# UoB-HPC/pbf-sph

Hardware: AMD Instinct MI355X
Metric: particle-steps/sec (1 M particles, 4 iters) + achieved HBM GB/s, 1/2/4/8 MI355X (higher is better)
Workload: dtype f32; 1 GPU; dam-break, 1024000 particles (nominal 1048576), box 4600^3, h=0.1, K=4, dt=0.01245, scale=500; timed = simulation frames [200, 2687) after 195 settle + 5 warm-up frames; particles=1024000, solver_iter=4, settle_frames=195, math=precise (IEEE div/sqrt, no contraction), parallelism=1 GPU, device-resident

## Files before the change

### pbf-sph_amd/csrc/pbf_hip.hip

```cpp
#include "pbf_hip.h"

#include <hip/hip_runtime.h>

#include <cmath>
#include <cstdio>
#include <cstdlib>
#include <cstring>
#include <algorithm>
#include <atomic>
#include <initializer_list>
#include <limits>
#include <map>
#include <string>
#include <utility>
#include <vector>

#include "pbf_kernels.hpp"
#include "pbf_slab.hpp"
#include "pbf_tiles.hpp"
#include "pbf_mc.hpp"
#include "pbf_whitewater.hpp"
#include "pbf_anisotropy.hpp"
#include "pbf_aniso_field.hpp"
#include "pbf_mesh_sdf.hpp"
// ... 44 lines not shown
  ~Pinned() { reset(); }
  void reset() {
    if (p) (void)hipHostFree(p);
    p = nullptr, count = 0;
  }
  hipError_t ensure(size_t n, bool zero = true) {
    if (count >= n) return hipSuccess;
    reset();
    const hipError_t e = hipHostMalloc(reinterpret_cast<void **>(&p), n * sizeof(T), hipHostMallocDefault);
    if (e != hipSuccess) {
      p = nullptr;
      return e;
    }
    if (zero) std::memset(static_cast<void *>(p), 0, n * sizeof(T));
    count = n;
    return hipSuccess;
  }
};

template <typename T> struct Mailbox {
  Pinned<T> rec;
  uint32_t seq = 0;
  hipError_t arm(uint32_t &word) {
    word = ++seq ? seq : ++seq;
    return rec.ensure(1);
  }
};
struct SceneRecord {
  uint32_t kept, seq;
};

constexpr uint32_t kTickets = 252;
constexpr uint32_t kCtlWords = kTickets + 4;
constexpr int kBrickZ = 4;

enum Stage { ST_PREDICT = 0, ST_SORT, ST_DIFFUSE, ST_LAMBDA, ST_DELTA, ST_FINALISE, ST_BUILD, ST_COUNT };
const char *kStageNames[ST_COUNT] = {"advect+zindex",      "sortz+gridtable", "sph-diffuse",
                                     "sph-lambda",         "sph-delta",       "sph-finalise",
                                     "sph-lambda/list-build"};

struct EventPair {
  hipEvent_t a, b;
  int stage;
};

}

struct StepState {
  DerivedState st;
  bool hasObstacles;
  uint32_t tableN, gatherSeq;
  uint64_t extent[3];
  double minExtent[3];
  void *bufs[15];
  size_t caps[15];
};
struct GraphEntry {
  hipGraphExec_t exec = nullptr;
  StepState after;
};
struct GraphKey {
  StepState before;
  unsigned char params[sizeof(double) * 11 + 32];
  uint64_t n;
  uint64_t collider;
  int options[10];
// ... 22 lines not shown
  bool ghostsPending = false;
  bool slabConfigured = false;
  pbf_slab_cut slabCut{0, 0, 0, 0};
  uint32_t xoff = 0;
  int32_t shiftL = 0, shiftR = 0;
  pbf_comm *comm = nullptr;
  std::vector<uint32_t> cuts;
  uint32_t capMig = 0, capGhost = 0;
  uint32_t wireCap = 0;
  DevBuf wireSend[2], wireRecv[2];
  DevBuf wireGhost[2];
  bool slabStepMode = false;
  size_t sortLive = 0;
  uint32_t ghostAt = 0;
  uint32_t slabSeq = 0;
  uint64_t slabHostSyncs = 0;
  Pinned<uint32_t> hostCounts;
  size_t reserve = 0;
  uint32_t nOwned = 0, sentL = 0, sentR = 0, gotL = 0, gotR = 0;
  DevBuf latticePN, latticeC, mcCounts, mcOffsets, mcSums, meshV, meshN, meshC, mcNear;
  Pinned<char> meshHost;
  bool meshStaged = false;
  uint64_t mcSample[3] = {0, 0, 0};
  uint64_t mcTriangles = 0;
  DevBuf mcEdgeWord, mcEdgeOffsets, mcEdgeSums, meshT;
  enum MeshKind { MESH_NONE, MESH_SOUP, MESH_INDEXED };
  MeshKind meshKind = MESH_NONE;
  uint64_t mcVertices = 0;
  DevBuf qpos;
  DevBuf nbrList, nbrCount;
  int rowMajor = 1;
  DevBuf rowPstar[2], rowMass, rowQpos, rowXYZ, rowType, rowSlotOf, linTable, linSums;
  DevBuf rowCol, rowMortonOf, rowSegs;
  uint32_t rowSegShift = 0;
  uint32_t diffuseCap = 0;
  int rowDiffuse = 1;
  uint32_t rowShift = 0;
  uint64_t nbrExtraAt = 0;
  uint32_t nbrChunks = 0, nbrChunksOpt = 0;
  double cohesion = 0, adhesion = 0;
  DevBuf surfA, surfB;
  ColliderState col;
  SolidLattice<DevBuf> solid[2];
  DevBuf colliderPose;
  DevBuf pushRec, pushCtl, pushPartials, pushOut;
  Mailbox<WrenchRecord> hostWrench;
  DevBuf bodyRec;
  Mailbox<BodyStateRecord> hostBody;
  DevBuf frictionRec, frictionCtl, frictionPartials;
  Mailbox<WrenchRecord> hostFriction;
  bool sdfCull = true;
  uint64_t sdfLaunchPairs = 0;
  std::vector<pbf_source> sources;
  std::vector<pbf_drain> drains;
  uint32_t emitTotal = 0;
  size_t uploaded = 0;
  DevBuf sceneSources, sceneDrains, drainCounts;
  Mailbox<SceneRecord> hostScene;
  uint64_t sceneHostSyncs = 0;
  DevBuf queryPoints, queryCounts, queryIds;
  DevBuf samplePoints, sampleOut;
  DevBuf diagRho, diagNbr, diagPartials;
  Mailbox<DiagRecord> hostDiag;
  uint64_t diagRhoAt = 0;
  uint64_t orderEpoch = 1;
  bool wwOn = false;
// ... 1 lines not shown
  uint64_t wwFrame = 0;
  size_t wwCount = 0;
  int wwCur = 0;
  DevBuf wwPos[2], wwVel[2], wwKind[2], wwParent[2];
  DevBuf wwSample, wwAlive, wwAliveOff, wwSums, wwFieldA, wwFieldB, wwPot, wwEmit, wwOffset, wwChildKind;
  Mailbox<WwRecord> hostWw;
  uint64_t wwPotAt = 0;
  DevBuf anisoOut;
  DevBuf anisoRec;
  void *regPtr = nullptr;
  size_t regBytes = 0;
  size_t stagedBytes = 0;
  int graphMode = 0;
  std::map<GraphKey, GraphEntry> graphs;
  uint64_t allocEpoch = 0;
  uint32_t graphMisses = 0;
  uint64_t graphReplays = 0, graphCaptures = 0;
  pbf_params lastParams{};
  bool haveParams = false;
  bool reuseLists = true;
  int splitBuild = 8;
  int pipeline = -1;
  int coop = 0;
  bool fusePredict = true;
  bool cellDiffuse = true;
  bool overlapDiffuse = true;
  bool overlapDiffuseForced = false;
  hipStream_t sideStream = nullptr;
  hipStream_t copyStream = nullptr;
  hipEvent_t evPacked = nullptr;
  bool downloadPending = false;
  hipEvent_t evFork = nullptr, evJoin = nullptr;
  bool diffusePending = false;
  DevBuf diffSum, diffCnt;
  bool fuseDiffuse = false;
  bool fuseNextPredict = false;
  DevBuf bricks, brickCtl;
  DevBuf bigCells;
  uint32_t gatherSeq = 0;
  int numCUs = 256;
  uint32_t timingMask = 0xFFFFFFFFu;
  uint32_t padLds = 0;
  std::map<const void *, size_t> ldsLimit;
  int gatherKind = 1;
  uint32_t tileCap = 0, listMax = 0;
  size_t tableCap = 0;
  uint32_t tableN = 0;
  uint64_t extent[3] = {0, 0, 0};
  double minExtent[3] = {0, 0, 0};

  std::vector<EventPair> pending;
  std::vector<hipEvent_t> freeEvents;
  double stageMs[ST_COUNT] = {0};
  uint64_t stageCalls[ST_COUNT] = {0};
};

namespace {

#define HIPCHK(ctx, expr)                                                                          \
  do {                                                                                             \
    hipError_t e_ = (expr);                                                                        \
    if (e_ != hipSuccess) {                                                                        \
      (ctx)->err = std::string(#expr) + ": " + hipGetErrorString(e_);                              \
      return PBF_ERR_HIP;                                                                          \
    }                                                                                              \
  } while (0)

int fail(pbf_ctx *ctx, int code, const std::string &msg) {
  ctx->err = msg;
  return code;
}

int ensure(pbf_ctx *ctx, DevBuf &b, size_t bytes, bool zero = false) {
  if (b.cap >= bytes) return PBF_OK;
  DevBuf fresh;
  fresh.cap = bytes + bytes / 4 + 256;
  HIPCHK(ctx, hipMalloc(&fresh.p, fresh.cap));
  ctx->allocEpoch++;
  if (zero) HIPCHK(ctx, hipMemsetAsync(fresh.p, 0, fresh.cap, ctx->stream));
  if (b.p) {
    HIPCHK(ctx, hipStreamSynchronize(ctx->stream));
    HIPCHK(ctx, b.reset());
  }
  b = std::move(fresh);
  return PBF_OK;
}

bool record_current(const pbf_ctx *ctx, uint64_t madeAt) { return madeAt == ctx->orderEpoch && ctx->st.sorted; }

template <typename N> size_t vsz() { return sizeof(vec4<N>); }

int ensure_particles(pbf_ctx *ctx, size_t n) {
  n = std::max(n, ctx->reserve);
  if (ctx->cap >= n) return PBF_OK;
  if (ctx->reserve) n += n / 4 + 65536;
  const size_t v = ctx->fp64 ? sizeof(double4) : sizeof(float4);
  for (int s = 0; s < 2; ++s) {
    if (int rc = ensure(ctx, ctx->pos4[s], n * v)) return rc;
    if (int rc = ensure(ctx, ctx->vel4[s], n * v)) return rc;
    if (int rc = ensure(ctx, ctx->col4[s], n * v)) return rc;
    if (int rc = ensure(ctx, ctx->id[s], n * 8)) return rc;
    if (int rc = ensure(ctx, ctx->type[s], n)) return rc;
    if (int rc = ensure(ctx, ctx->key[s], n * 4)) return rc;
  }
  for (int s = 0; s < 3; ++s)
    if (int rc = ensure(ctx, ctx->pstar[s], n * v)) return rc;
  if (int rc = ensure(ctx, ctx->permTmp, n * 4)) return rc;
// ... 57 lines not shown
  }
  if (ctx->slabConfigured) {
    c.xoff = ctx->xoff;
    const uint64_t hi = ctx->slabCut.has_right ? std::min<uint64_t>(ext[0], uint64_t(ctx->slabCut.xhi) + 1) : ext[0];
    ext[0] = hi > ctx->xoff ? hi - ctx->xoff : 1;
  }
  c.tableN = morton_encode(uint32_t(ext[0]), uint32_t(ext[1]), uint32_t(ext[2]));
  if (c.tableN == 0) return fail(ctx, PBF_ERR_INVALID, "empty grid (max_bound <= min_bound?)");
  c.poly6Factor = poly6_factor<N>(h);
  c.spikyFactor = spiky_factor<N>(h);
  {
    const N r = N(CorrDeltaQ * h);
    const N d = (h * h) - r * r;
    c.p6DeltaQ = r <= h ? c.poly6Factor * (d * d * d) : N(0);
  }
  c.diffuseT = c.dt / N(750.0);
  c.h2filter = (h * h) * N(1.00001);
  c.n = uint32_t(ctx->n);
  c.nWells = uint32_t(p->n_wells > 0 ? p->n_wells : 0);
  c.hasObstacles = ctx->hasObstacles ? 1u : 0u;
  ctx->tableN = c.tableN;
  return PBF_OK;
}

int drop_histogram(pbf_ctx *ctx) {
  if (ctx->st.counted && ctx->count.p) HIPCHK(ctx, hipMemsetAsync(ctx->count.p, 0, ctx->count.cap, ctx->stream));
  ctx->st.histogram_dropped();
  return PBF_OK;
}

int ensure_table(pbf_ctx *ctx, uint32_t tableN) {
  const size_t entries = size_t(tableN) + 2;
  if (ctx->tableCap >= entries) return PBF_OK;
  if (ctx->count.p) {
    HIPCHK(ctx, hipStreamSynchronize(ctx->stream));
    HIPCHK(ctx, ctx->count.reset());
  }
  if (int rc = ensure(ctx, ctx->count, (entries + SCAN_TILE) * 4, true)) return rc;
  if (int rc = ensure(ctx, ctx->table, (entries + SCAN_TILE) * 4)) return rc;
  const size_t nb = (entries + SCAN_TILE - 1) / SCAN_TILE + 1;
  if (int rc = ensure(ctx, ctx->blockSums, nb * 4)) return rc;
  if (int rc = ensure(ctx, ctx->bricks, (entries / Brick<kBrickZ>::HOME + 2) * 4)) return rc;
  if (int rc = ensure(ctx, ctx->brickCtl, kCtlWords * 4)) return rc;
  ctx->tableCap = ctx->count.cap / 4 - SCAN_TILE;
  return PBF_OK;
}

hipEvent_t get_event(pbf_ctx *ctx) {
  if (!ctx->freeEvents.empty()) {
    hipEvent_t e = ctx->freeEvents.back();
    ctx->freeEvents.pop_back();
    return e;
  }
  hipEvent_t e = nullptr;
  (void)hipEventCreate(&e);
  return e;
}
int resolve_events(pbf_ctx *ctx) {
  if (ctx->pending.empty()) return PBF_OK;
  HIPCHK(ctx, hipStreamSynchronize(ctx->stream));
  for (auto &ep : ctx->pending) {
    float ms = 0.f;
    if (hipEventElapsedTime(&ms, ep.a, ep.b) == hipSuccess) {
      ctx->stageMs[ep.stage] += ms;
      ctx->stageCalls[ep.stage] += 1;
    }
    ctx->freeEvents.push_back(ep.a);
    ctx->freeEvents.push_back(ep.b);
  }
  ctx->pending.clear();
  return PBF_OK;
}
struct StageTimer {
  pbf_ctx *ctx;
  EventPair ep{};
  bool on;
// ... 83 lines not shown
  return PBF_OK;
}

bool row_mode(const pbf_ctx *ctx);

void brick_list(pbf_ctx *ctx, uint32_t tableN, bool counterIsZero = false) {
  if (ctx->st.bricksValid) return;
  if (!counterIsZero) (void)hipMemsetAsync(ctx->brickCtl.p, 0, 4, ctx->stream);
  const uint32_t home = Brick<kBrickZ>::HOME, nBricks = (tableN + home - 1) / home;
  hipLaunchKernelGGL(k_brick_list, grid_for(nBricks), dim3(BLOCK), 0, ctx->stream, ctx->table.as<const uint32_t>(), tableN, home,
                     nBricks, ctx->bricks.as<uint32_t>(), ctx->brickCtl.as<uint32_t>());
  ctx->st.bricks_listed();
}

void launch_scans(pbf_ctx *ctx, const ScanJobs &jobs, int njobs, uint32_t *zero = nullptr, uint32_t nZero = 0) {
  const uint32_t blocks = jobs.nb[0] + (njobs > 1 ? jobs.nb[1] : 0u);
  hipLaunchKernelGGL(k_scan_block_sums, dim3(blocks), dim3(BLOCK), 0, ctx->stream, jobs);
  hipLaunchKernelGGL(k_scan_sums, dim3(uint32_t(njobs)), dim3(BLOCK), 0, ctx->stream, jobs, zero, nZero);
  hipLaunchKernelGGL(k_scan_apply, dim3(blocks), dim3(BLOCK), 0, ctx->stream, jobs);
}
ScanJobs scan_job(const uint32_t *count, uint32_t len, uint32_t *sums, uint32_t *table) {
  ScanJobs j{};
  j.count[0] = count, j.sums[0] = sums, j.table[0] = table, j.len[0] = len, j.nb[0] = (len + SCAN_TILE - 1) / SCAN_TILE;
  return j;
}

int ensure_reaction(pbf_ctx *ctx);
template <typename N> int stage_sort(pbf_ctx *ctx, const pbf_params *p) {
  if (!ctx->st.counted) return fail(ctx, PBF_ERR_STATE, "pbf_stage_sort needs pbf_stage_predict first");
  StepConsts<N> c;
  if (int rc = make_consts<N>(ctx, p, c)) return rc;
  if (c.tableN != ctx->st.countedTableN) return fail(ctx, PBF_ERR_STATE, "bounds changed between predict and sort");
  StageTimer t(ctx, ST_SORT);
  const uint32_t len = c.tableN + 2;
  uint32_t *count = ctx->count.as<uint32_t>(), *table = ctx->table.as<uint32_t>(),
           *sums = ctx->blockSums.as<uint32_t>();
  ScanJobs jobs = scan_job(count, len, sums, table);
  int njobs = 1;
  const int s = ctx->st.cur, d = 1 - s;
  uint32_t *ctl = ctx->brickCtl.as<uint32_t>();
  RowArrays<N> row{};
  const bool rows = row_mode(ctx), rowDiffuse = rows && ctx->cellDiffuse && ctx->rowDiffuse > 0;
  if (rows) {
    uint32_t pshift = 1;
    while (pshift < 10 && (uint64_t(1) << (3 * pshift)) < uint64_t(c.tableN)) ++pshift;
    const size_t ncells = size_t(1) << (3 * pshift), llen = ncells + 1;
    const uint32_t lnb = uint32_t((llen + SCAN_TILE - 1) / SCAN_TILE);
    const size_t v = sizeof(vec4<N>);
    if (int rc = ensure(ctx, ctx->linTable, (ncells + 2 + SCAN_TILE) * 4)) return rc;
    if (int rc = ensure(ctx, ctx->linSums, (size_t(lnb) + 2) * 4)) return rc;
    for (int k = 0; k < 2; ++k)
      if (int rc = ensure(ctx, ctx->rowPstar[k], ctx->cap * v)) return rc;
    if (int rc = ensure(ctx, ctx->rowMass, ctx->cap * sizeof(N))) return rc;
    if (int rc = ensure(ctx, ctx->rowQpos, (ctx->cap + QPOS_PAD) * 8)) return rc;
    if (int rc = ensure(ctx, ctx->rowXYZ, ctx->cap * 4)) return rc;
    if (int rc = ensure(ctx, ctx->rowType, ctx->cap)) return rc;
    if (int rc = ensure(ctx, ctx->rowSlotOf, ctx->cap * 4)) return rc;
    const uint32_t segShift = std::min<uint32_t>(pshift, 6u);
    const size_t nSegTotal = ncells >> segShift;
    if (rowDiffuse) {
      if (int rc = ensure(ctx, ctx->rowCol, ctx->cap * v)) return rc;
      if (int rc = ensure(ctx, ctx->rowMortonOf, ctx->cap * 4)) return rc;
      if (int rc = ensure(ctx, ctx->rowSegs, (std::min(nSegTotal, ctx->cap) + 1) * 4)) return rc;
    }
    jobs.count[1] = nullptr, jobs.rowShift = pshift, jobs.tableN = c.tableN;
    jobs.sums[1] = ctx->linSums.as<uint32_t>(), jobs.table[1] = ctx->linTable.as<uint32_t>();
    jobs.len[1] = uint32_t(llen), jobs.nb[1] = lnb;
    njobs = 2;
    if (rowDiffuse)
      jobs.segs = ctx->rowSegs.as<uint32_t>(), jobs.nSegs = ctl + kTickets + 3, jobs.segShift = segShift;
    launch_scans(ctx, jobs, njobs, ctl, kCtlWords);
    row = RowArrays<N>{ctx->rowPstar[0].as<vec4<N>>(), ctx->rowMass.as<N>(), ctx->rowQpos.as<uint2>(), ctx->rowXYZ.as<uint32_t>(),
                       ctx->rowType.as<uint8_t>(), ctx->rowSlotOf.as<uint32_t>(),
                       rowDiffuse ? ctx->rowCol.as<vec4<N>>() : nullptr, rowDiffuse ? ctx->rowMortonOf.as<uint32_t>() : nullptr,
                       ctx->linTable.as<const uint32_t>(), ctl + kTickets + 2, pshift};
    ctx->rowShift = pshift, ctx->rowSegShift = segShift;
  }
  if (njobs == 1) launch_scans(ctx, jobs, 1, ctl, kCtlWords);
  uint32_t *nBig = ctl + kTickets + 1;
  if (int rc = ensure(ctx, ctx->bigCells, (ctx->cap / BIG_CELL + 2) * 4)) return rc;
  hipLaunchKernelGGL(k_scatter_slots, grid_for(ctx->n), dim3(BLOCK), 0, ctx->stream, c.n, c.tableN,
                     ctx->key[s].as<const uint32_t>(), table, ctx->cellSlot.as<const uint32_t>(), count,
                     ctx->permTmp.as<uint32_t>(),
                     ctx->bigCells.as<uint32_t>(), nBig);
  hipLaunchKernelGGL(k_sort_big_cells, dim3(64), dim3(BLOCK), 0, ctx->stream, table, c.tableN,
                     ctx->bigCells.as<const uint32_t>(), nBig, ctx->permTmp.as<uint32_t>(),
                     ctx->key[s].as<const uint32_t>());
  const size_t nLive = ctx->slabStepMode ? ctx->sortLive : ctx->n;
  hipLaunchKernelGGL((k_rank_move<N>), grid_for(nLive), dim3(BLOCK), 0, ctx->stream, c, uint32_t(nLive), c.tableN,
                     ctx->permTmp.as<const uint32_t>(), table, arrays<N>(ctx, s, s), arrays<N>(ctx, d, d),
                     ctx->slabActive ? ctx->slotOf.as<uint32_t>() : nullptr, ctx->qpos.as<uint2>(), row);
  LAUNCH_CHECK(ctx);
  ctx->n = nLive;
  ctx->gatherSeq = 0;
  ctx->st.sorted_now(rows, rowDiffuse);
  ctx->orderEpoch++;
  if (ctx->col.reaction) {
    if (int rc = ensure_reaction(ctx)) return rc;
    const uint32_t n2 = 2u * uint32_t(ctx->n);
    hipLaunchKernelGGL((k_push_clear<N>), grid_for(std::max<size_t>(n2, 1)), dim3(BLOCK), 0, ctx->stream, n2, ctx->pushRec.as<vec4<N>>(),
                       ctx->pushCtl.as<unsigned long long>());
    LAUNCH_CHECK(ctx);
    ctx->col.records_cleared(ctx->orderEpoch);
  }
  if (!rowDiffuse) brick_list(ctx, c.tableN, true);
  return PBF_OK;
}

inline int other_pstar(const pbf_ctx *ctx) { return ctx->st.pcur == 2 ? ctx->st.cur : 2; }

enum GatherMode { GATHER_PLAIN = 0, GATHER_SAVE_LISTS = 1, GATHER_FROM_LISTS = 2 };

bool row_offsets_fit(const pbf_ctx *ctx) { return uint64_t(ctx->n) * (ctx->fp64 ? sizeof(vec4<double>) : sizeof(vec4<float>)) <= ROW_BYTES_MAX; }
bool row_mode(const pbf_ctx *ctx) {
  return ctx->rowMajor > 0 && ctx->gatherKind == 1 && ctx->splitBuild == 8 && ctx->coop == 0 && ctx->reuseLists &&
         !ctx->fuseDiffuse && ctx->graphMode <= 0 &&
         !(ctx->desc.flags & PBF_FLAG_NO_LDS) && row_offsets_fit(ctx);
}
template <typename N> RowWalk row_walk(pbf_ctx *ctx) {
  return RowWalk{ctx->linTable.as<const uint32_t>(), ctx->rowXYZ.as<const uint32_t>(), ctx->rowSlotOf.as<const uint32_t>(),
                 ctx->table.as<const uint32_t>(), ctx->tableN, ctx->rowShift};
// ... 140 lines not shown
        if (ctx->splitBuild == 4)
          launch_build_lists<N, Lists, 2, 16, FW>(ctx, c, only, ps, qp, args.type, key, table);
        else
          switch (ctx->listMax ? ctx->listMax : 32u) {
            case 16: launch_build_lists<N, Lists, 4, 16, FW>(ctx, c, only, ps, qp, args.type, key, table); break;
            case 24: launch_build_lists<N, Lists, 4, 24, FW>(ctx, c, only, ps, qp, args.type, key, table); break;
            default: launch_build_lists<N, Lists, 4, 32, FW>(ctx, c, only, ps, qp, args.type, key, table); break;
          }
      }
      from_lists();
    } else if (mode == GATHER_SAVE_LISTS) {
      hipLaunchKernelGGL((k_gather_lists<N, Op, 16, true>), g, b, 0, ctx->stream, c, args, key, table, nbr_lists(ctx, true));
    } else {
      switch (ctx->listMax ? ctx->listMax : 16u) {
        case 12: hipLaunchKernelGGL((k_gather_lists<N, Op, 12>), g, b, 0, ctx->stream, c, args, key, table, nbr_lists(ctx, false)); break;
        case 24: hipLaunchKernelGGL((k_gather_lists<N, Op, 24>), g, b, 0, ctx->stream, c, args, key, table, nbr_lists(ctx, false)); break;
        case 32: hipLaunchKernelGGL((k_gather_lists<N, Op, 32>), g, b, 0, ctx->stream, c, args, key, table, nbr_lists(ctx, false)); break;
        default: hipLaunchKernelGGL((k_gather_lists<N, Op, 16>), g, b, 0, ctx->stream, c, args, key, table, nbr_lists(ctx, false)); break;
      }
    }
    LAUNCH_CHECK(ctx);
    return PBF_OK;
  }
  return fail(ctx, PBF_ERR_INVALID, "unknown gather kind");
}

int join_diffuse(pbf_ctx *ctx) {
  if (!ctx->diffusePending) return PBF_OK;
  ctx->diffusePending = false;
  HIPCHK(ctx, hipStreamWaitEvent(ctx->stream, ctx->evJoin, 0));
  return PBF_OK;
}

template <typename N> int stage_diffuse(pbf_ctx *ctx, const pbf_params *p, bool overlap = false) {
  StepConsts<N> c;
  if (int rc = make_consts<N>(ctx, p, c)) return rc;
  const int s = ctx->st.cur, d = 1 - s;
  typename DiffuseOp<N>::Args args{ctx->col4[s].as<const vec4<N>>(), ctx->col4[d].as<vec4<N>>(),
                                   ctx->type[s].as<const uint8_t>()};
  const bool timed = (ctx->desc.flags & PBF_FLAG_STAGE_TIMING) != 0 && ((ctx->timingMask >> ST_DIFFUSE) & 1u) != 0;
  overlap = overlap && ctx->overlapDiffuse && ctx->cellDiffuse && !(ctx->desc.flags & PBF_FLAG_NO_LDS) && !timed &&
            (ctx->overlapDiffuseForced || ctx->n >= (size_t(1) << 19));
  bool parked = false;
  StageTimer t(ctx, ST_DIFFUSE);
  if (ctx->cellDiffuse && ctx->st.diffuse_on_rows() && ctx->rowDiffuse) {
    const uint32_t cap = ctx->diffuseCap ? ctx->diffuseCap : 640u;
    const size_t lds = size_t(cap + 8) * sizeof(vec4<N>) + size_t(DIFFUSE_ROW_THREADS) * (4 * sizeof(N) + 4) + cap + 8;
    if (int rc = raise_lds_limit(ctx, reinterpret_cast<const void *>(k_diffuse_rows<N>), lds)) return rc;
    const uint32_t perCU = uint32_t(std::max<size_t>(1, std::min<size_t>(16, (160 * 1024) / (lds + 256))));
    const uint32_t blocks = std::max(8u, (uint32_t(ctx->numCUs) * perCU) & ~7u);
    hipLaunchKernelGGL((k_diffuse_rows<N>), dim3(blocks), dim3(DIFFUSE_ROW_THREADS), lds, ctx->stream, c,
                       row_walk<N>(ctx), ctx->rowCol.as<const vec4<N>>(), ctx->rowType.as<const uint8_t>(),
                       ctx->rowMortonOf.as<const uint32_t>(), ctx->rowSegs.as<const uint32_t>(),
                       ctx->brickCtl.as<const uint32_t>() + kTickets + 3, ctx->rowSegShift, args.colOut, cap, uint32_t(ctx->n));
    LAUNCH_CHECK(ctx);
  } else if (ctx->cellDiffuse && !(ctx->desc.flags & PBF_FLAG_NO_LDS)) {
    brick_list(ctx, c.tableN);
    vec4<N> *cellSum = ctx->pstar[other_pstar(ctx)].as<vec4<N>>();
    uint32_t *cellCnt = ctx->nbrCount.as<uint32_t>();
    hipStream_t st = ctx->stream;
    uint32_t cap = 3072u;
    if (overlap) cap = 2048u;
    const size_t lds = Brick<4>::HDR + size_t(cap) * sizeof(vec4<N>);
    uint32_t perCU = uint32_t((160 * 1024) / (lds + 1024));
    if (overlap) {
      if (int rc = ensure(ctx, ctx->diffSum, ctx->cap * sizeof(vec4<N>))) return rc;
      if (int rc = ensure(ctx, ctx->diffCnt, ctx->cap * 4)) return rc;
      if (!ctx->sideStream) {
        HIPCHK(ctx, hipStreamCreateWithFlags(&ctx->sideStream, hipStreamNonBlocking));
        HIPCHK(ctx, hipEventCreateWithFlags(&ctx->evFork, hipEventDisableTiming));
        HIPCHK(ctx, hipEventCreateWithFlags(&ctx->evJoin, hipEventDisableTiming));
      }
      cellSum = ctx->diffSum.as<vec4<N>>(), cellCnt = ctx->diffCnt.as<uint32_t>();
      st = ctx->sideStream;
      perCU = 1;
      HIPCHK(ctx, hipEventRecord(ctx->evFork, ctx->stream));
      HIPCHK(ctx, hipStreamWaitEvent(st, ctx->evFork, 0));
    }
    const uint32_t *key = ctx->key[s].as<const uint32_t>(), *table = ctx->table.as<const uint32_t>();
    static_assert(kBrickZ == 4, "the sort stage's brick list is the 4 x 4 x 4 one");
    hipLaunchKernelGGL((k_diffuse_bricks<N>), dim3(uint32_t(ctx->numCUs) * perCU), dim3(DIFFUSE_BRICK_THREADS), lds,
                       st, c, args.colIn, args.type, table, ctx->bricks.as<const uint32_t>(),
                       ctx->brickCtl.as<const uint32_t>(), cellSum, cellCnt, cap);
    hipLaunchKernelGGL((k_diffuse_apply<N>), grid_for(ctx->n), dim3(BLOCK), 0, st, c, args, key, table,
                       cellSum, cellCnt);
    LAUNCH_CHECK(ctx);
    if (overlap) {
      HIPCHK(ctx, hipEventRecord(ctx->evJoin, st));
      ctx->diffusePending = true;
    }
    parked = !overlap;
  } else if (int rc = launch_gather<N, DiffuseOp<N>>(ctx, c, args)) {
    return rc;
  }
  std::swap(ctx->col4[s], ctx->col4[d]);
  ctx->st.diffused(parked);
  return PBF_OK;
}

#ifndef PBF_ROWS_W
#define PBF_ROWS_W 4
#endif
#ifndef PBF_ROWS_LMAX
#define PBF_ROWS_LMAX 32
#endif
// ... 201 lines not shown
    if (int rc = launch_gather<N, XsphOp<N, FAST>>(ctx, c, a3)) return rc;
    std::swap(ctx->vel4[s], ctx->vel4[o]);
  }
  if (surface_on(ctx))
    if (int rc = surface_tension_impl<N, FAST>(ctx, c)) return rc;
  ctx->st.extras_done(p->vorticity != 0, surface_on(ctx));
  return PBF_OK;
}
template <typename N> int extras(pbf_ctx *ctx, const pbf_params *p, const StepConsts<N> &c) {
  if (ctx->slabActive && surface_on(ctx))
    return fail(ctx, PBF_ERR_STATE, "surface tension is not supported in slab mode (pbf_set_surface_tension(ctx, 0, 0) turns it off)");
  if (ctx->slabActive) return PBF_OK;
  return DISPATCH_FAST(ctx, extras_impl, ctx, p, c);
}

template <typename N> int stage_friction(pbf_ctx *ctx, const pbf_params *p) {
  const uint32_t n = uint32_t(ctx->n), nb = (n + DIAG_TILE - 1) / DIAG_TILE;
  const int s = ctx->st.cur;
  const pbf_collider_friction *rec = ctx->frictionRec.as<const pbf_collider_friction>();
  const double *vw = ctx->col.body ? ctx->bodyRec.as<const colliderbody::Record>()->st.velocity : rec->velocity;
  hipLaunchKernelGGL((k_collider_friction<N>), dim3(nb), dim3(BLOCK), 0, ctx->stream, n, N(p->scale), N(p->dt), rec, vw,
                     ctx->colliderPose.as<const ColliderPose<N>>(), ctx->pushRec.as<const vec4<N>>(), push_slots(ctx),
                     ctx->pos4[s].as<const vec4<N>>(), ctx->vel4[s].as<vec4<N>>(), ctx->frictionPartials.as<WrenchPartial>(),
                     ctx->frictionCtl.as<colliderfriction::Ctl>());
  LAUNCH_CHECK(ctx);
  ctx->col.friction_passed();
  return PBF_OK;
}

template <typename N> int stage_finalise(pbf_ctx *ctx, const pbf_params *p) {
  StepConsts<N> c;
  if (int rc = make_consts<N>(ctx, p, c)) return rc;
  const int s = ctx->st.cur;
  if (ctx->col.friction) {
    if (int rc = collider_refuse_slab(ctx)) return rc;
    if (!push_current(ctx)) return fail(ctx, PBF_ERR_STATE, "the collider friction needs a sort since the reaction records were enabled");
  }
  if (ctx->fuseNextPredict && !extras_on(ctx, p) && !ctx->col.friction) {
    ctx->fuseNextPredict = false;
    if (int rc = ensure_table(ctx, c.tableN)) return rc;
    if (int rc = drop_histogram(ctx)) return rc;
    if (int rc = upload_wells(ctx, p)) return rc;
    if (int rc = join_diffuse(ctx)) return rc;
    StageTimer t(ctx, ST_FINALISE);
    std::swap(ctx->pstar[ctx->st.pcur], ctx->pstar[s]);
    hipLaunchKernelGGL((k_finalise_predict<N>), grid_for(ctx->n), dim3(BLOCK), 0, ctx->stream, c,
                       ctx->type[s].as<const uint8_t>(), ctx->pstar[s].as<vec4<N>>(), ctx->pos4[s].as<vec4<N>>(),
                       ctx->vel4[s].as<vec4<N>>(), ctx->wells.as<const N>(), ctx->key[s].as<uint32_t>(),
                       ctx->count.as<uint32_t>(), ctx->cellSlot.as<uint32_t>(), ctx->rowPstar[ctx->st.rcur].as<const vec4<N>>(),
                       ctx->st.pstarInRows ? ctx->rowSlotOf.as<const uint32_t>() : nullptr);
    ctx->st.predicted(c.tableN, true);
    LAUNCH_CHECK(ctx);
    return PBF_OK;
  }
  ctx->fuseNextPredict = false;
  if (ctx->st.pstarInRows && extras_on(ctx, p))
    if (int rc = materialise_pstar<N>(ctx)) return rc;
  StageTimer t(ctx, ST_FINALISE);
  if (ctx->st.pstarInRows)
    hipLaunchKernelGGL((k_finalise<N>), grid_for(ctx->n), dim3(BLOCK), 0, ctx->stream, c, ctx->type[s].as<const uint8_t>(),
                       ctx->rowPstar[ctx->st.rcur].as<const vec4<N>>(), ctx->pos4[s].as<vec4<N>>(), ctx->vel4[s].as<vec4<N>>(),
                       ctx->rowSlotOf.as<const uint32_t>());
  else
    hipLaunchKernelGGL((k_finalise<N>), grid_for(ctx->n), dim3(BLOCK), 0, ctx->stream, c, ctx->type[s].as<const uint8_t>(),
                       ctx->pstar[ctx->st.pcur].as<const vec4<N>>(), ctx->pos4[s].as<vec4<N>>(), ctx->vel4[s].as<vec4<N>>(),
                       static_cast<const uint32_t *>(nullptr));
  LAUNCH_CHECK(ctx);
  std::swap(ctx->pstar[ctx->st.pcur], ctx->pstar[s]);
  ctx->st.finalised();
  if (ctx->col.friction)
    if (int rc = stage_friction<N>(ctx, p)) return rc;
  if (extras_on(ctx, p)) return extras<N>(ctx, p, c);
  return PBF_OK;
}

bool scene_on(const pbf_ctx *ctx) { return !ctx->sources.empty() || !ctx->drains.empty(); }
const char *kSceneSlabError = "sources and drains are not supported in slab mode (pbf_set_sources / pbf_set_drains with n = 0 clear them)";

template <typename N> int stage_scene(pbf_ctx *ctx, const pbf_params *p) {
  if (!scene_on(ctx)) return PBF_OK;
  if (ctx->comm || ctx->slabActive || ctx->ghostsPending) return fail(ctx, PBF_ERR_STATE, kSceneSlabError);
  const size_t e = ctx->emitTotal;
  const size_t limit = ctx->reserve ? std::min(ctx->cap, std::max(ctx->reserve, ctx->uploaded)) : ctx->cap;
  if (ctx->n + e > limit)
    return fail(ctx, PBF_ERR_INVALID, "particle capacity exceeded by the sources' emission: call pbf_reserve before pbf_upload");
  if (e == 0 && (ctx->drains.empty() || ctx->n == 0)) return PBF_OK;
  if (ctx->downloadPending) (void)pbf_download_aos_end(ctx);
  if (int rc = join_diffuse(ctx)) return rc;
  if (int rc = drop_histogram(ctx)) return rc;
  const int s = ctx->st.cur;
// ... 26 lines not shown
    LAUNCH_CHECK(ctx);
    ctx->st.compacted(true);
  }
  ctx->n = kept;
  return PBF_OK;
}

template <typename N> int stage_body(pbf_ctx *ctx, const pbf_params *p) {
  if (int rc = collider_refuse_slab(ctx)) return rc;
  if (!push_current(ctx)) return fail(ctx, PBF_ERR_STATE, "the collider body needs a sort since the reaction records were enabled");
  const uint32_t n = uint32_t(ctx->n), nb = (n + DIAG_TILE - 1) / DIAG_TILE;
  hipLaunchKernelGGL((k_wrench_partial<N>), dim3(nb), dim3(BLOCK), 0, ctx->stream, n, ctx->pushRec.as<const vec4<N>>(), push_slots(ctx),
                     ctx->pos4[ctx->st.cur].as<const vec4<N>>(), ctx->pushPartials.as<WrenchPartial>());
  if (ctx->col.friction)
    hipLaunchKernelGGL((k_body_kick_advance<N>), dim3(1), dim3(BLOCK), 0, ctx->stream, ctx->frictionPartials.as<const WrenchPartial>(),
                       ctx->frictionCtl.as<colliderfriction::Ctl>(), nb, ctx->pushPartials.as<const WrenchPartial>(), double(p->dt),
                       ctx->bodyRec.as<colliderbody::Record>(), ctx->colliderPose.as<ColliderPose<N>>());
  else
    hipLaunchKernelGGL((k_body_advance<N>), dim3(1), dim3(BLOCK), 0, ctx->stream, nb, ctx->pushPartials.as<const WrenchPartial>(),
                       double(p->dt), ctx->bodyRec.as<colliderbody::Record>(), ctx->colliderPose.as<ColliderPose<N>>());
  LAUNCH_CHECK(ctx);
  return PBF_OK;
}

template <typename N> int step_impl(pbf_ctx *ctx, const pbf_params *p) {
  if (scene_on(ctx))
    if (int rc = stage_scene<N>(ctx, p)) return rc;
  if (ctx->n == 0) return PBF_OK;
  if (!ctx->st.take_prediction())
    if (int rc = stage_predict<N>(ctx, p)) return rc;
  if (int rc = stage_sort<N>(ctx, p)) return rc;
  const bool fuse = ctx->fuseDiffuse && p->iteration > 0 && ctx->gatherKind == 1 && ctx->reuseLists &&
                    !(ctx->desc.flags & PBF_FLAG_NO_LDS);
  if (!fuse) {
    if (int rc = stage_diffuse<N>(ctx, p, p->iteration > 0)) return rc;
  }
  for (uint64_t it = 0; it < p->iteration; ++it) {
    if (int rc = stage_lambda<N>(ctx, p, fuse && it == 0)) return rc;
    if (int rc = stage_delta<N>(ctx, p)) return rc;
  }
  if (ctx->col.body)
    if (int rc = stage_body<N>(ctx, p)) return rc;
  if (int rc = stage_finalise<N>(ctx, p)) return rc;
  return join_diffuse(ctx);
}

int check(pbf_ctx *ctx, const pbf_params *p, bool needSorted) {
  if (!ctx) return PBF_ERR_INVALID;
  if (!p) return fail(ctx, PBF_ERR_INVALID, "params == NULL");
  if (!(p->scale > 0) || !(p->dt > 0)) return fail(ctx, PBF_ERR_INVALID, "dt and scale must be > 0");
  if (needSorted && !ctx->st.sorted) return fail(ctx, PBF_ERR_STATE, "stage needs pbf_stage_sort first");
  HIPCHK(ctx, hipSetDevice(ctx->device));
  ctx->lastParams = *p;
  ctx->haveParams = true;
  return PBF_OK;
}

struct Refuse {
  pbf_ctx *ctx;
  const char *who;
  int params(const pbf_params *p) const {
    if (!(p->scale > 0) || !(p->dt > 0)) return fail(ctx, PBF_ERR_INVALID, "dt and scale must be > 0");
    return PBF_OK;
  }
  int slab_mode() const {
    if (ctx->comm || ctx->slabActive || ctx->ghostsPending || ctx->slabConfigured)
      return fail(ctx, PBF_ERR_STATE, std::string(who) + " is not supported in slab mode");
    return PBF_OK;
  }
  int no_step(const char *part = "") const {
    if (!ctx->st.sorted) return fail(ctx, PBF_ERR_STATE, std::string(who) + part + " needs a step first (no valid cell table)");
    return PBF_OK;
  }
};

int drop_ghosts(pbf_ctx *ctx);
// ... 451 lines not shown
  }
  GraphEntry entry;
  const hipError_t ei = hipGraphInstantiate(&entry.exec, graph, nullptr, nullptr, 0);
  (void)hipGraphDestroy(graph);
  if (ei != hipSuccess) {
    (void)hipGetLastError();
    ctx->graphMode = 0;
    restore(ctx, before);
    ctx->diffusePending = false;
    return DISPATCH(ctx, step_impl, ctx, p);
  }
  entry.after = snapshot(ctx);
  ctx->graphs.emplace(key, entry);
  ctx->graphCaptures++, ctx->graphMisses++;
  HIPCHK(ctx, hipGraphLaunch(entry.exec, ctx->stream));
  return PBF_OK;
}

}

extern "C" {

int pbf_steps(pbf_ctx *ctx, const pbf_params *p, uint32_t count) {
  if (int rc = check(ctx, p, false)) return rc;
  if (int rc = drop_ghosts(ctx)) return rc;
  const bool timed = (ctx->desc.flags & PBF_FLAG_STAGE_TIMING) != 0 &&
                     (((ctx->timingMask >> ST_PREDICT) & 1u) != 0 || ((ctx->timingMask >> ST_FINALISE) & 1u) != 0);
  const bool fusable = ctx->fusePredict && !timed && ctx->graphMode <= 0 && !ctx->slabActive && ctx->n != 0 && !scene_on(ctx);
  for (uint32_t i = 0; i < count; ++i) {
    ctx->fuseNextPredict = fusable && i + 1 < count;
    if (int rc = step_maybe_graphed(ctx, p)) {
      ctx->fuseNextPredict = false;
      (void)ctx->st.take_prediction();
      return rc;
    }
  }
  ctx->fuseNextPredict = false;
  return PBF_OK;
}
int pbf_graph_stats(const pbf_ctx *ctx, uint64_t out[3]) {
  if (!ctx || !out) return PBF_ERR_INVALID;
  out[0] = ctx->graphCaptures, out[1] = ctx->graphReplays, out[2] = uint64_t(ctx->graphMode > 0);
  return PBF_OK;
}
int pbf_sync(pbf_ctx *ctx) {
  if (!ctx) return PBF_ERR_INVALID;
  HIPCHK(ctx, hipSetDevice(ctx->device));
  HIPCHK(ctx, hipStreamSynchronize(ctx->stream));
  return PBF_OK;
}

int pbf_stage_predict(pbf_ctx *ctx, const pbf_params *p) {
  if (int rc = check(ctx, p, false)) return rc;
  if (ctx->n == 0) return PBF_OK;
  return DISPATCH(ctx, stage_predict, ctx, p);
}
int pbf_stage_sort(pbf_ctx *ctx, const pbf_params *p) {
  if (int rc = check(ctx, p, false)) return rc;
  if (ctx->n == 0) return PBF_OK;
  return DISPATCH(ctx, stage_sort, ctx, p);
}
int pbf_stage_diffuse(pbf_ctx *ctx, const pbf_params *p) {
  if (int rc = check(ctx, p, true)) return rc;
  return DISPATCH(ctx, stage_diffuse, ctx, p);
}
int pbf_stage_lambda(pbf_ctx *ctx, const pbf_params *p) {
  if (int rc = check(ctx, p, true)) return rc;
  return DISPATCH(ctx, stage_lambda, ctx, p);
}
int pbf_stage_delta(pbf_ctx *ctx, const pbf_params *p) {
  if (ctx && (collider_on(ctx) || scenery_on(ctx)))
// ... 2054 lines not shown
```

### pbf-sph_amd/csrc/pbf_kernels.hpp

```cpp
#pragma once

#include <type_traits>

#include "pbf_collider.hpp"
#include "pbf_collider_body.hpp"
#include "pbf_common.hpp"

namespace pbf {

constexpr int BLOCK = 256;

template <typename N> __device__ inline int64_t cell_coord(N v) {
  return static_cast<int64_t>(v);
}

template <typename F> __device__ inline void wave_bucket_atomic(uint32_t bucket, F &&leader_op, uint32_t &before, uint32_t &rank) {
  const uint32_t lane = threadIdx.x & 63u;
  const uint64_t below = (1ull << lane) - 1ull;
  bool pending = true;
  uint32_t cnt = 0, leader = lane;
  rank = 0;
  while (__any(pending)) {
    if (pending) {
      const uint32_t b = __builtin_amdgcn_readfirstlane(bucket);
// ... 148 lines not shown
#pragma unroll
    for (uint32_t k = 0; k < SCAN_ITEMS; ++k) {
      const uint32_t lin = base + k, z = lin >> (2u * ps);
      const uint32_t code = morton_encode(lin & mask, (lin >> ps) & mask, z);
      v[k] = (z <= mask && code + 1u < jobs.tableN) ? count[code] : 0u;
    }
  }
}
__global__ __launch_bounds__(BLOCK) void k_scan_block_sums(ScanJobs jobs) {
  const uint32_t j = blockIdx.x >= jobs.nb[0] ? 1u : 0u, blk = blockIdx.x - (j ? jobs.nb[0] : 0u);
  const uint32_t *__restrict__ count = jobs.count[j];
  const uint32_t len = jobs.len[j];
  const uint32_t base = blk * SCAN_TILE + threadIdx.x * SCAN_ITEMS;
  uint32_t s = 0;
  if (j && jobs.rowShift) {
    uint32_t v[SCAN_ITEMS];
    row_populations(jobs, base, v);
#pragma unroll
    for (int k = 0; k < SCAN_ITEMS; ++k) s += v[k];
  } else if (base + SCAN_ITEMS <= len) {
    const uint4 a = *reinterpret_cast<const uint4 *>(count + base);
    const uint4 b = *reinterpret_cast<const uint4 *>(count + base + 4);
    s = a.x + a.y + a.z + a.w + b.x + b.y + b.z + b.w;
  } else {
    for (int k = 0; k < SCAN_ITEMS; ++k)
      if (base + k < len) s += count[base + k];
  }
  uint32_t total;
  block_excl_scan(s, &total);
  if (threadIdx.x == 0) jobs.sums[j][blk] = total;
}

__global__ __launch_bounds__(BLOCK) void k_scan_sums(ScanJobs jobs, uint32_t *__restrict__ zero, uint32_t nZero) {
  if (blockIdx.x == 0)
    for (uint32_t k = threadIdx.x; k < nZero; k += BLOCK) zero[k] = 0u;
  uint32_t *__restrict__ blockSums = jobs.sums[blockIdx.x];
  const uint32_t nb = jobs.nb[blockIdx.x];
  uint32_t carry = 0;
  for (uint32_t base = 0; base < nb; base += BLOCK) {
    const uint32_t i = base + threadIdx.x;
    const uint32_t v = i < nb ? blockSums[i] : 0u;
    uint32_t total;
    const uint32_t ex = block_excl_scan(v, &total);
    if (i < nb) blockSums[i] = carry + ex;
    carry += total;
  }
}

__global__ __launch_bounds__(BLOCK) void k_scan_apply(ScanJobs jobs) {
  const uint32_t j = blockIdx.x >= jobs.nb[0] ? 1u : 0u, blk = blockIdx.x - (j ? jobs.nb[0] : 0u);
  const uint32_t *__restrict__ count = jobs.count[j];
  uint32_t *__restrict__ table = jobs.table[j];
  const uint32_t len = jobs.len[j];
  const uint32_t base = blk * SCAN_TILE + threadIdx.x * SCAN_ITEMS;
  uint32_t v[SCAN_ITEMS];
  uint32_t s = 0;
  if (j && jobs.rowShift) {
    row_populations(jobs, base, v);
#pragma unroll
    for (int k = 0; k < SCAN_ITEMS; ++k) s += v[k];
  } else {
#pragma unroll
    for (int k = 0; k < SCAN_ITEMS; ++k) {
      v[k] = (base + k < len) ? count[base + k] : 0u;
      s += v[k];
    }
  }
  if (j && jobs.segs) {
// ... 2705 lines not shown
```

Baseline: 899.5 million particle-steps/s.

## Defer row diffusion onto side stream to overlap with finalise and next step

Moves the viscosity/diffuse pass off the critical path: when eligible (large N, no stage timing, no graphs or slabs), diffusion is launched on a side stream at finalise time and joined only before the next sort's rank-move kernel. To make that safe, the cell table, linear table and row segment buffers are double-buffered with a parity-selected segment counter, so the next sort can rebuild them while the deferred diffuse still reads the old ones. This adds extra buffer memory, event sync and more complex error/join handling, and the concurrent kernels compete for bandwidth.

```diff
diff --git a/pbf-sph_amd/csrc/pbf_hip.hip b/pbf-sph_amd/csrc/pbf_hip.hip
--- a/pbf-sph_amd/csrc/pbf_hip.hip
+++ b/pbf-sph_amd/csrc/pbf_hip.hip
@@ -100,6 +100,7 @@
 
 constexpr uint32_t kTickets = 252;
 constexpr uint32_t kCtlWords = kTickets + 4;
+constexpr uint32_t kSegWord = kTickets + 3;
 constexpr int kBrickZ = 4;
 
 enum Stage { ST_PREDICT = 0, ST_SORT, ST_DIFFUSE, ST_LAMBDA, ST_DELTA, ST_FINALISE, ST_BUILD, ST_COUNT };
@@ -188,6 +189,8 @@
   int rowMajor = 1;
   DevBuf rowPstar[2], rowMass, rowQpos, rowXYZ, rowType, rowSlotOf, linTable, linSums;
   DevBuf rowCol, rowMortonOf, rowSegs;
+  DevBuf tablePrev, linTablePrev, rowSegsPrev;
+  uint32_t segParity = 0;
   uint32_t rowSegShift = 0;
   uint32_t diffuseCap = 0;
   int rowDiffuse = 1;
@@ -255,6 +258,8 @@
   bool downloadPending = false;
   hipEvent_t evFork = nullptr, evJoin = nullptr;
   bool diffusePending = false;
+  bool deferDiffuse = false;
+  bool diffuseCarried = false;
   DevBuf diffSum, diffCnt;
   bool fuseDiffuse = false;
   bool fuseNextPredict = false;
@@ -294,8 +299,11 @@
   return code;
 }
 
+int join_diffuse(pbf_ctx *ctx);
 int ensure(pbf_ctx *ctx, DevBuf &b, size_t bytes, bool zero = false) {
   if (b.cap >= bytes) return PBF_OK;
+  if (b.p)
+    if (int rc = join_diffuse(ctx)) return rc;
   DevBuf fresh;
   fresh.cap = bytes + bytes / 4 + 256;
   HIPCHK(ctx, hipMalloc(&fresh.p, fresh.cap));
@@ -419,16 +427,18 @@
 int ensure_table(pbf_ctx *ctx, uint32_t tableN) {
   const size_t entries = size_t(tableN) + 2;
   if (ctx->tableCap >= entries) return PBF_OK;
+  if (int rc = join_diffuse(ctx)) return rc;
   if (ctx->count.p) {
     HIPCHK(ctx, hipStreamSynchronize(ctx->stream));
     HIPCHK(ctx, ctx->count.reset());
   }
   if (int rc = ensure(ctx, ctx->count, (entries + SCAN_TILE) * 4, true)) return rc;
   if (int rc = ensure(ctx, ctx->table, (entries + SCAN_TILE) * 4)) return rc;
+  if (int rc = ensure(ctx, ctx->tablePrev, (entries + SCAN_TILE) * 4)) return rc;
   const size_t nb = (entries + SCAN_TILE - 1) / SCAN_TILE + 1;
   if (int rc = ensure(ctx, ctx->blockSums, nb * 4)) return rc;
   if (int rc = ensure(ctx, ctx->bricks, (entries / Brick<kBrickZ>::HOME + 2) * 4)) return rc;
-  if (int rc = ensure(ctx, ctx->brickCtl, kCtlWords * 4)) return rc;
+  if (int rc = ensure(ctx, ctx->brickCtl, (kCtlWords + 1) * 4)) return rc;
   ctx->tableCap = ctx->count.cap / 4 - SCAN_TILE;
   return PBF_OK;
 }
@@ -578,6 +588,8 @@
   if (int rc = make_consts<N>(ctx, p, c)) return rc;
   if (c.tableN != ctx->st.countedTableN) return fail(ctx, PBF_ERR_STATE, "bounds changed between predict and sort");
   StageTimer t(ctx, ST_SORT);
+  std::swap(ctx->table, ctx->tablePrev), std::swap(ctx->linTable, ctx->linTablePrev), std::swap(ctx->rowSegs, ctx->rowSegsPrev);
+  ctx->segParity ^= 1u;
   const uint32_t len = c.tableN + 2;
   uint32_t *count = ctx->count.as<uint32_t>(), *table = ctx->table.as<uint32_t>(),
            *sums = ctx->blockSums.as<uint32_t>();
@@ -594,6 +606,7 @@
     const uint32_t lnb = uint32_t((llen + SCAN_TILE - 1) / SCAN_TILE);
     const size_t v = sizeof(vec4<N>);
     if (int rc = ensure(ctx, ctx->linTable, (ncells + 2 + SCAN_TILE) * 4)) return rc;
+    if (int rc = ensure(ctx, ctx->linTablePrev, (ncells + 2 + SCAN_TILE) * 4)) return rc;
     if (int rc = ensure(ctx, ctx->linSums, (size_t(lnb) + 2) * 4)) return rc;
     for (int k = 0; k < 2; ++k)
       if (int rc = ensure(ctx, ctx->rowPstar[k], ctx->cap * v)) return rc;
@@ -608,21 +621,22 @@
       if (int rc = ensure(ctx, ctx->rowCol, ctx->cap * v)) return rc;
       if (int rc = ensure(ctx, ctx->rowMortonOf, ctx->cap * 4)) return rc;
       if (int rc = ensure(ctx, ctx->rowSegs, (std::min(nSegTotal, ctx->cap) + 1) * 4)) return rc;
+      if (int rc = ensure(ctx, ctx->rowSegsPrev, (std::min(nSegTotal, ctx->cap) + 1) * 4)) return rc;
     }
     jobs.count[1] = nullptr, jobs.rowShift = pshift, jobs.tableN = c.tableN;
     jobs.sums[1] = ctx->linSums.as<uint32_t>(), jobs.table[1] = ctx->linTable.as<uint32_t>();
     jobs.len[1] = uint32_t(llen), jobs.nb[1] = lnb;
     njobs = 2;
     if (rowDiffuse)
-      jobs.segs = ctx->rowSegs.as<uint32_t>(), jobs.nSegs = ctl + kTickets + 3, jobs.segShift = segShift;
-    launch_scans(ctx, jobs, njobs, ctl, kCtlWords);
+      jobs.segs = ctx->rowSegs.as<uint32_t>(), jobs.nSegs = ctl + kSegWord + ctx->segParity, jobs.segShift = segShift;
+    launch_scans(ctx, jobs, njobs, ctl, kSegWord);
     row = RowArrays<N>{ctx->rowPstar[0].as<vec4<N>>(), ctx->rowMass.as<N>(), ctx->rowQpos.as<uint2>(), ctx->rowXYZ.as<uint32_t>(),
                        ctx->rowType.as<uint8_t>(), ctx->rowSlotOf.as<uint32_t>(),
                        rowDiffuse ? ctx->rowCol.as<vec4<N>>() : nullptr, rowDiffuse ? ctx->rowMortonOf.as<uint32_t>() : nullptr,
                        ctx->linTable.as<const uint32_t>(), ctl + kTickets + 2, pshift};
     ctx->rowShift = pshift, ctx->rowSegShift = segShift;
   }
-  if (njobs == 1) launch_scans(ctx, jobs, 1, ctl, kCtlWords);
+  if (njobs == 1) launch_scans(ctx, jobs, 1, ctl, kSegWord);
   uint32_t *nBig = ctl + kTickets + 1;
   if (int rc = ensure(ctx, ctx->bigCells, (ctx->cap / BIG_CELL + 2) * 4)) return rc;
   hipLaunchKernelGGL(k_scatter_slots, grid_for(ctx->n), dim3(BLOCK), 0, ctx->stream, c.n, c.tableN,
@@ -633,6 +647,7 @@
                      ctx->bigCells.as<const uint32_t>(), nBig, ctx->permTmp.as<uint32_t>(),
                      ctx->key[s].as<const uint32_t>());
   const size_t nLive = ctx->slabStepMode ? ctx->sortLive : ctx->n;
+  if (int rc = join_diffuse(ctx)) return rc;
   hipLaunchKernelGGL((k_rank_move<N>), grid_for(nLive), dim3(BLOCK), 0, ctx->stream, c, uint32_t(nLive), c.tableN,
                      ctx->permTmp.as<const uint32_t>(), table, arrays<N>(ctx, s, s), arrays<N>(ctx, d, d),
                      ctx->slabActive ? ctx->slotOf.as<uint32_t>() : nullptr, ctx->qpos.as<uint2>(), row);
@@ -839,6 +854,50 @@
   return PBF_OK;
 }
 
+int ensure_side_stream(pbf_ctx *ctx) {
+  if (ctx->sideStream) return PBF_OK;
+  HIPCHK(ctx, hipStreamCreateWithFlags(&ctx->sideStream, hipStreamNonBlocking));
+  HIPCHK(ctx, hipEventCreateWithFlags(&ctx->evFork, hipEventDisableTiming));
+  HIPCHK(ctx, hipEventCreateWithFlags(&ctx->evJoin, hipEventDisableTiming));
+  return PBF_OK;
+}
+
+template <typename N> int launch_diffuse_rows(pbf_ctx *ctx, const StepConsts<N> &c, hipStream_t st) {
+  const int s = ctx->st.cur, d = 1 - s;
+  const uint32_t cap = ctx->diffuseCap ? ctx->diffuseCap : 640u;
+  const size_t lds = size_t(cap + 8) * sizeof(vec4<N>) + size_t(DIFFUSE_ROW_THREADS) * (4 * sizeof(N) + 4) + cap + 8;
+  if (int rc = raise_lds_limit(ctx, reinterpret_cast<const void *>(k_diffuse_rows<N>), lds)) return rc;
+  const uint32_t perCU = uint32_t(std::max<size_t>(1, std::min<size_t>(16, (160 * 1024) / (lds + 256))));
+  const uint32_t blocks = std::max(8u, (uint32_t(ctx->numCUs) * perCU) & ~7u);
+  hipLaunchKernelGGL((k_diffuse_rows<N>), dim3(blocks), dim3(DIFFUSE_ROW_THREADS), lds, st, c,
+                     row_walk<N>(ctx), ctx->rowCol.as<const vec4<N>>(), ctx->rowType.as<const uint8_t>(),
+                     ctx->rowMortonOf.as<const uint32_t>(), ctx->rowSegs.as<const uint32_t>(),
+                     ctx->brickCtl.as<const uint32_t>() + kSegWord + ctx->segParity, ctx->rowSegShift,
+                     ctx->col4[d].as<vec4<N>>(), cap, uint32_t(ctx->n));
+  LAUNCH_CHECK(ctx);
+  std::swap(ctx->col4[s], ctx->col4[d]);
+  ctx->st.diffused(false);
+  return PBF_OK;
+}
+
+constexpr size_t kDeferDiffuseMin = size_t(1) << 19;
+bool defers_diffuse(const pbf_ctx *ctx) {
+  const bool timed = (ctx->desc.flags & PBF_FLAG_STAGE_TIMING) != 0 && ((ctx->timingMask >> ST_DIFFUSE) & 1u) != 0;
+  return ctx->overlapDiffuse && ctx->cellDiffuse && ctx->rowDiffuse && ctx->st.diffuse_on_rows() && !timed &&
+         ctx->graphMode <= 0 && !ctx->slabActive && !ctx->slabStepMode &&
+         (ctx->overlapDiffuseForced || ctx->n >= kDeferDiffuseMin);
+}
+
+template <typename N> int fork_diffuse(pbf_ctx *ctx, const StepConsts<N> &c) {
+  if (int rc = ensure_side_stream(ctx)) return rc;
+  HIPCHK(ctx, hipEventRecord(ctx->evFork, ctx->stream));
+  HIPCHK(ctx, hipStreamWaitEvent(ctx->sideStream, ctx->evFork, 0));
+  const int rc = launch_diffuse_rows<N>(ctx, c, ctx->sideStream);
+  HIPCHK(ctx, hipEventRecord(ctx->evJoin, ctx->sideStream));
+  ctx->diffusePending = true;
+  return rc;
+}
+
 template <typename N> int stage_diffuse(pbf_ctx *ctx, const pbf_params *p, bool overlap = false) {
   StepConsts<N> c;
   if (int rc = make_consts<N>(ctx, p, c)) return rc;
@@ -851,16 +910,7 @@
   bool parked = false;
   StageTimer t(ctx, ST_DIFFUSE);
   if (ctx->cellDiffuse && ctx->st.diffuse_on_rows() && ctx->rowDiffuse) {
-    const uint32_t cap = ctx->diffuseCap ? ctx->diffuseCap : 640u;
-    const size_t lds = size_t(cap + 8) * sizeof(vec4<N>) + size_t(DIFFUSE_ROW_THREADS) * (4 * sizeof(N) + 4) + cap + 8;
-    if (int rc = raise_lds_limit(ctx, reinterpret_cast<const void *>(k_diffuse_rows<N>), lds)) return rc;
-    const uint32_t perCU = uint32_t(std::max<size_t>(1, std::min<size_t>(16, (160 * 1024) / (lds + 256))));
-    const uint32_t blocks = std::max(8u, (uint32_t(ctx->numCUs) * perCU) & ~7u);
-    hipLaunchKernelGGL((k_diffuse_rows<N>), dim3(blocks), dim3(DIFFUSE_ROW_THREADS), lds, ctx->stream, c,
-                       row_walk<N>(ctx), ctx->rowCol.as<const vec4<N>>(), ctx->rowType.as<const uint8_t>(),
-                       ctx->rowMortonOf.as<const uint32_t>(), ctx->rowSegs.as<const uint32_t>(),
-                       ctx->brickCtl.as<const uint32_t>() + kTickets + 3, ctx->rowSegShift, args.colOut, cap, uint32_t(ctx->n));
-    LAUNCH_CHECK(ctx);
+    return launch_diffuse_rows<N>(ctx, c, ctx->stream);
   } else if (ctx->cellDiffuse && !(ctx->desc.flags & PBF_FLAG_NO_LDS)) {
     brick_list(ctx, c.tableN);
     vec4<N> *cellSum = ctx->pstar[other_pstar(ctx)].as<vec4<N>>();
@@ -873,11 +923,7 @@
     if (overlap) {
       if (int rc = ensure(ctx, ctx->diffSum, ctx->cap * sizeof(vec4<N>))) return rc;
       if (int rc = ensure(ctx, ctx->diffCnt, ctx->cap * 4)) return rc;
-      if (!ctx->sideStream) {
-        HIPCHK(ctx, hipStreamCreateWithFlags(&ctx->sideStream, hipStreamNonBlocking));
-        HIPCHK(ctx, hipEventCreateWithFlags(&ctx->evFork, hipEventDisableTiming));
-        HIPCHK(ctx, hipEventCreateWithFlags(&ctx->evJoin, hipEventDisableTiming));
-      }
+      if (int rc = ensure_side_stream(ctx)) return rc;
       cellSum = ctx->diffSum.as<vec4<N>>(), cellCnt = ctx->diffCnt.as<uint32_t>();
       st = ctx->sideStream;
       perCU = 1;
@@ -1145,6 +1191,8 @@
   StepConsts<N> c;
   if (int rc = make_consts<N>(ctx, p, c)) return rc;
   const int s = ctx->st.cur;
+  const bool fork = ctx->deferDiffuse;
+  ctx->deferDiffuse = false;
   if (ctx->col.friction) {
     if (int rc = collider_refuse_slab(ctx)) return rc;
     if (!push_current(ctx)) return fail(ctx, PBF_ERR_STATE, "the collider friction needs a sort since the reaction records were enabled");
@@ -1154,7 +1202,12 @@
     if (int rc = ensure_table(ctx, c.tableN)) return rc;
     if (int rc = drop_histogram(ctx)) return rc;
     if (int rc = upload_wells(ctx, p)) return rc;
-    if (int rc = join_diffuse(ctx)) return rc;
+    if (!fork) {
+      if (int rc = join_diffuse(ctx)) return rc;
+    } else {
+      if (int rc = fork_diffuse<N>(ctx, c)) return rc;
+      ctx->diffuseCarried = true;
+    }
     StageTimer t(ctx, ST_FINALISE);
     std::swap(ctx->pstar[ctx->st.pcur], ctx->pstar[s]);
     hipLaunchKernelGGL((k_finalise_predict<N>), grid_for(ctx->n), dim3(BLOCK), 0, ctx->stream, c,
@@ -1169,6 +1222,8 @@
   ctx->fuseNextPredict = false;
   if (ctx->st.pstarInRows && extras_on(ctx, p))
     if (int rc = materialise_pstar<N>(ctx)) return rc;
+  if (fork)
+    if (int rc = fork_diffuse<N>(ctx, c)) return rc;
   StageTimer t(ctx, ST_FINALISE);
   if (ctx->st.pstarInRows)
     hipLaunchKernelGGL((k_finalise<N>), grid_for(ctx->n), dim3(BLOCK), 0, ctx->stream, c, ctx->type[s].as<const uint8_t>(),
@@ -1261,7 +1316,8 @@
   if (int rc = stage_sort<N>(ctx, p)) return rc;
   const bool fuse = ctx->fuseDiffuse && p->iteration > 0 && ctx->gatherKind == 1 && ctx->reuseLists &&
                     !(ctx->desc.flags & PBF_FLAG_NO_LDS);
-  if (!fuse) {
+  const bool defer = !fuse && defers_diffuse(ctx);
+  if (!fuse && !defer) {
     if (int rc = stage_diffuse<N>(ctx, p, p->iteration > 0)) return rc;
   }
   for (uint64_t it = 0; it < p->iteration; ++it) {
@@ -1270,7 +1326,17 @@
   }
   if (ctx->col.body)
     if (int rc = stage_body<N>(ctx, p)) return rc;
-  if (int rc = stage_finalise<N>(ctx, p)) return rc;
+  ctx->deferDiffuse = defer;
+  ctx->diffuseCarried = false;
+  const int rc = stage_finalise<N>(ctx, p);
+  ctx->deferDiffuse = false;
+  if (rc) {
+    const std::string why = ctx->err;
+    (void)join_diffuse(ctx);
+    ctx->err = why;
+    return rc;
+  }
+  if (ctx->diffuseCarried) return PBF_OK;
   return join_diffuse(ctx);
 }
 
@@ -1788,11 +1854,14 @@
     if (int rc = step_maybe_graphed(ctx, p)) {
       ctx->fuseNextPredict = false;
       (void)ctx->st.take_prediction();
+      const std::string why = ctx->err;
+      (void)join_diffuse(ctx);
+      ctx->err = why;
       return rc;
     }
   }
   ctx->fuseNextPredict = false;
-  return PBF_OK;
+  return join_diffuse(ctx);
 }
 int pbf_graph_stats(const pbf_ctx *ctx, uint64_t out[3]) {
   if (!ctx || !out) return PBF_ERR_INVALID;
diff --git a/pbf-sph_amd/csrc/pbf_kernels.hpp b/pbf-sph_amd/csrc/pbf_kernels.hpp
--- a/pbf-sph_amd/csrc/pbf_kernels.hpp
+++ b/pbf-sph_amd/csrc/pbf_kernels.hpp
@@ -204,8 +204,10 @@
 }
 
 __global__ __launch_bounds__(BLOCK) void k_scan_sums(ScanJobs jobs, uint32_t *__restrict__ zero, uint32_t nZero) {
-  if (blockIdx.x == 0)
+  if (blockIdx.x == 0) {
     for (uint32_t k = threadIdx.x; k < nZero; k += BLOCK) zero[k] = 0u;
+    if (threadIdx.x == 0 && jobs.segs) *jobs.nSegs = 0u;
+  }
   uint32_t *__restrict__ blockSums = jobs.sums[blockIdx.x];
   const uint32_t nb = jobs.nb[blockIdx.x];
   uint32_t carry = 0;
```

New measurement: 898.4 million particle-steps/s. About the same (-0.1%).
